# StuLiu/RegDA

Measured on AMD Instinct MI355X. Metric: src+tgt 512x512 image-pairs/sec (SSL step), higher is better.
Workload: dtype bf16; 1 GPU; st.regda.2potsdam SSL step, resnet101 DeepLabV2(PPM), batch 8+8 512x512 per GPU, online EMA teacher; global_batch=8, parallelism=dp1

## Files before the change

regda_amd/csrc/conv_kernels.hip:

```cpp
#include <stdio.h>
#include <stdlib.h>
#include <string.h>

#include "common.h"
#include <type_traits>
#include <vector>

struct ConvArgs {
    const bf16_t* x;
    const bf16_t* w;
    bf16_t* y;
    const bf16_t* res;
    rgda_stat_t* stats;
    int ldx, ldy, ldres;
    int N, H, W, Cin, Ho, Wo, Cout, KH, KW, stride, pad, dil, mode;
    int M;
    int tiles_c, tiles_p;
    int rows_per_group;
    int howo_shift, wo_shift;
    unsigned long long* dbg;
    int tpw;
    int skip;
    const unsigned char* res_mask;
    const bf16_t* bn_y;
// ... 1509 lines not shown
    const int nj1 = (t + 256) / SWP, nx1 = (t + 256) % SWP;
    const bool second = t + 256 < 2 * SWP;
    float na0[3] = {0.f, 0.f, 0.f}, na1[3] = {0.f, 0.f, 0.f}, nb0[3] = {0.f, 0.f, 0.f}, nb1[3] = {0.f, 0.f, 0.f};
    if (1 < rpw) {
        load_px(7 + nj0, nx0, na0);
        if (second) load_px(7 + nj1, nx1, na1);
    }
    float s[8], q[8];
#pragma unroll
    for (int e = 0; e < 8; ++e) { s[e] = 0.f; q[e] = 0.f; }
    EpiParams P;
    epilogue_params<KIND>(a, ((n * Ho + ho0) * Wo + wo0), (t % (BC / 8)) * 8, true, P);
    for (int r = 0; r < rpw; ++r) {
        const int ho = ho0 + r;
        asm volatile("s_waitcnt lgkmcnt(0)" ::: "memory");
        __builtin_amdgcn_s_barrier();
        if (r + 2 < rpw) {
            load_px(2 * r + 9 + nj0, nx0, nb0);
            if (second) load_px(2 * r + 9 + nj1, nx1, nb1);
        }
        f32x16 acc[1][1], acc1;
#pragma unroll
        for (int e = 0; e < 16; ++e) { acc[0][0][e] = 0.f; acc1[e] = 0.f; }
        const int px = wp * 32 + lrow;
        const unsigned char* fbase = srow + px * 16 + lk * 16;
        const int s0 = (2 * r) % 7;
#pragma unroll
        for (int kh = 0; kh < 7; ++kh) {
            const int slot = (s0 + kh >= 7) ? s0 + kh - 7 : s0 + kh;
            const bf16x8 fb0 = *(const bf16x8*)(fbase + slot * SROW);
            const bf16x8 fb1 = *(const bf16x8*)(fbase + slot * SROW + 32);
            acc[0][0] = __builtin_amdgcn_mfma_f32_32x32x16_bf16(fa[kh][0], fb0, acc[0][0], 0, 0, 0);
            acc1 = __builtin_amdgcn_mfma_f32_32x32x16_bf16(fa[kh][1], fb1, acc1, 0, 0, 0);
        }
#pragma unroll
        for (int e = 0; e < 16; ++e) acc[0][0][e] += acc1[e];
        const int m0 = (n * Ho + ho) * Wo + wo0;
        conv_epilogue<BC, BP, WC, WP, true, KIND>(a, acc, se, m0, 0, s, q, r + 1 == rpw, blockIdx.x & (NREP - 1), &P);
        if (r + 1 < rpw) {
            store_px(2 * r + 7 + nj0, nx0, na0);
            if (second) store_px(2 * r + 7 + nj1, nx1, na1);
        }
#pragma unroll
        for (int c = 0; c < 3; ++c) { na0[c] = nb0[c]; na1[c] = nb1[c]; }
    }
#endif
}

static int stem_conv_launch(const float* img, const void* wgt, void* y, int ldy, rgda_stat_t* stats, int stat_groups,
                            const BnEvalFuse* bne, int N, int H, int W, int Ho, int Wo, rgda_stream_t stream) {
    if (!img || !wgt || !y || N <= 0 || H <= 0 || W <= 0 || (ldy & 7) || ldy < 64) return RGDA_ERR_ARG;
    if (Ho != (H + 6 - 7) / 2 + 1 || Wo != (W + 6 - 7) / 2 + 1) return RGDA_ERR_ARG;
    if (Wo % 64) return RGDA_ERR_UNSUPPORTED;
    if ((long long)3 * H * W >= (1ll << 28)) return RGDA_ERR_UNSUPPORTED;
    if (stat_groups < 1) stat_groups = 1;
    if ((N % stat_groups) || (bne && stats)) return RGDA_ERR_ARG;
    const long long M = (long long)N * Ho * Wo;
    if (M > 0x7fffffffLL) return RGDA_ERR_ARG;
    ConvArgs a;
    a.x = nullptr; a.w = (const bf16_t*)wgt; a.y = (bf16_t*)y; a.res = nullptr; a.stats = stats; a.res_mask = nullptr;
    a.ldx = 0; a.ldy = ldy; a.ldres = 0;
    a.N = N; a.H = H; a.W = W; a.Cin = 3; a.Ho = Ho; a.Wo = Wo; a.Cout = 64; a.KH = 7; a.KW = 7;
    a.stride = 2; a.pad = 3; a.dil = 1; a.mode = 0;
    a.M = (int)M; a.tiles_c = 1; a.tiles_p = 0;
    a.rows_per_group = (int)(M / stat_groups);
    a.howo_shift = a.wo_shift = -1; a.dbg = nullptr; a.tpw = 0; a.skip = 0;
    a.bn_y = a.bn_x = nullptr; a.bn_mask = nullptr; a.bn_mi = a.bn_nscale = nullptr; a.bn_ldy = a.bn_ldx = a.bn_rpi = a.bn_relu = 0;
    a.bn_gamma = a.bn_beta = nullptr; a.xf.stats = nullptr;
    a.ev_rm = a.ev_rv = a.ev_gamma = a.ev_beta = nullptr; a.ev_eps = 0.f; a.ev_relu = 0;
    if (bne) {
        if (!bne->rm || !bne->rv || !bne->gamma || !bne->beta) return RGDA_ERR_ARG;
        a.ev_rm = bne->rm; a.ev_rv = bne->rv; a.ev_gamma = bne->gamma; a.ev_beta = bne->beta; a.ev_eps = bne->eps; a.ev_relu = bne->relu;
    }
    int rpw = 8;
    if (const char* e = TUNE_ENV("RGDA_STEM_RPW")) rpw = atoi(e);
    else while (rpw < 64 && (long long)N * (Ho / (2 * rpw)) * (Wo / 64) >= 512 && !(Ho % (2 * rpw))) rpw *= 2;
    while (rpw > 1 && (Ho % rpw)) rpw >>= 1;
    const long long blocks = (long long)N * (Ho / rpw) * (Wo / 64);
    if (blocks > 0x7fffffffLL) return RGDA_ERR_ARG;
    if (bne) stem_conv_kernel<EPI_EV><<<(int)blocks, 256, 0, to_stream(stream)>>>(a, img, rpw);
    else if (stats) stem_conv_kernel<EPI_STATS><<<(int)blocks, 256, 0, to_stream(stream)>>>(a, img, rpw);
    else stem_conv_kernel<EPI_PLAIN><<<(int)blocks, 256, 0, to_stream(stream)>>>(a, img, rpw);
    RGDA_CHECK_LAUNCH();
    return RGDA_OK;
}

__global__ void __launch_bounds__(256) stem_wgrad_kernel(const float* __restrict__ img, const bf16_t* __restrict__ dy, int lddy,
                                                         float* __restrict__ part, int H, int W, int Ho, int Wo, int rpw) {
#if defined(__HIP_DEVICE_COMPILE__)
    constexpr int BP = 64, KP = 192;
    constexpr int SWP = 136, SROW = SWP * 8, NSLOT = 9;
    constexpr int DT = 64 * 128;
    __shared__ __attribute__((aligned(256))) unsigned char smem[2 * DT + NSLOT * SROW];
    unsigned char* const sd = smem;
    unsigned char* const srow = smem + 2 * DT;

    const int t = threadIdx.x, lane = t & 63;
    const int wave = __builtin_amdgcn_readfirstlane(t >> 6);
    const int wi = wave & 1, wj = wave >> 1;
    const int wtiles = Wo / BP, rblocks = Ho / rpw;
    const int wo0 = (blockIdx.x % wtiles) * BP;
    const int ho0 = ((blockIdx.x / wtiles) % rblocks) * rpw, n = blockIdx.x / (wtiles * rblocks);
    const int hbase = ho0 * 2 - 3;

    const size_t plane = (size_t)H * W;
    const float* const img_n = img + (size_t)n * 3 * plane;
    auto load_px = [&](int j, int x, float (&v)[3]) {
        const int hi = hbase + j, wcol = wo0 * 2 - 3 + x;
        const bool ok = (unsigned)hi < (unsigned)H && (unsigned)wcol < (unsigned)W && x < 134;
        const size_t o = (size_t)(ok ? hi : 0) * W + (ok ? wcol : 0);
#pragma unroll
        for (int c = 0; c < 3; ++c) v[c] = ok ? img_n[c * plane + o] : 0.f;
    };
    auto store_px = [&](int j, int x, const float (&v)[3]) {
        uint2 p;
        p.x = pack2bf(v[0], v[1]);
        p.y = pack2bf(v[2], 0.f);
        *(uint2*)(srow + (j % NSLOT) * SROW + x * 8) = p;
    };
    const int dpx = t >> 2, dq = t & 3;
    auto load_dy = [&](int ho, uint4& v0, uint4& v1) {
        const bf16_t* dp = dy + ((size_t)(n * Ho + ho) * Wo + wo0 + dpx) * lddy + dq * 16;
        v0 = *(const uint4*)dp;
        v1 = *(const uint4*)(dp + 8);
    };
    auto store_dy = [&](int buf, const uint4& v0, const uint4& v1) {
        const int f = (dpx >> 1) & 1, s0 = dq * 2, s1 = dq * 2 + 1;
        unsigned char* b = sd + buf * DT + dpx * 128;
        *(uint4*)(b + ((((s0 >> 2) ^ f) << 6) | ((s0 & 3) << 4))) = v0;
        *(uint4*)(b + ((((s1 >> 2) ^ f) << 6) | ((s1 & 3) << 4))) = v1;
    };
#pragma unroll
    for (int i = 0; i < 4; ++i) {
        const int idx = t + 256 * i;
        if (idx < 7 * SWP) {
            float v[3];
            load_px(idx / SWP, idx % SWP, v);
            store_px(idx / SWP, idx % SWP, v);
        }
    }
    {
        uint4 v0, v1;
        load_dy(ho0, v0, v1);
        store_dy(0, v0, v1);
    }
    const int nj0 = t / SWP, nx0 = t % SWP;
    const int nj1 = (t + 256) / SWP, nx1 = (t + 256) % SWP;
    const bool second = t + 256 < 2 * SWP;
    float na0[3] = {0.f, 0.f, 0.f}, na1[3] = {0.f, 0.f, 0.f}, nb0[3] = {0.f, 0.f, 0.f}, nb1[3] = {0.f, 0.f, 0.f};
    if (1 < rpw) {
        load_px(7 + nj0, nx0, na0);
        if (second) load_px(7 + nj1, nx1, na1);
    }
    const int g = lane >> 4, la = lane & 15;
    const int krow = (g >> 1) * 8 + (la >> 2);
    const int kcol2 = ((g & 1) * 16 + (la & 3) * 4) * 2;
    auto pack_tr = [](s16x4 lo, s16x4 hi) {
        u16x8 v8 = {(bf16_t)lo[0], (bf16_t)lo[1], (bf16_t)lo[2], (bf16_t)lo[3],
                    (bf16_t)hi[0], (bf16_t)hi[1], (bf16_t)hi[2], (bf16_t)hi[3]};
        return __builtin_bit_cast(bf16x8, v8);
    };
    auto tr_dy = [&](const unsigned char* base, int byte, int r0) {
        const int r1 = r0 + 4;
        const unsigned char* p0 = base + r0 * 128 + ((((byte >> 6) ^ ((r0 >> 1) & 1)) << 6) | (byte & 63));
        const unsigned char* p1 = base + r1 * 128 + ((((byte >> 6) ^ ((r1 >> 1) & 1)) << 6) | (byte & 63));
        return pack_tr(__builtin_amdgcn_ds_read_tr16_b64_v4i16((s16x4 __attribute__((address_space(3)))*)(p0)),
                       __builtin_amdgcn_ds_read_tr16_b64_v4i16((s16x4 __attribute__((address_space(3)))*)(p1)));
    };
    auto tr_img = [&](const unsigned char* rowbase, int r0) {
        const unsigned char* p0 = rowbase + r0 * 16 + kcol2;
        return pack_tr(__builtin_amdgcn_ds_read_tr16_b64_v4i16((s16x4 __attribute__((address_space(3)))*)(p0)),
                       __builtin_amdgcn_ds_read_tr16_b64_v4i16((s16x4 __attribute__((address_space(3)))*)(p0 + 64)));
    };
    f32x16 acc[4];
#pragma unroll
    for (int j = 0; j < 4; ++j)
#pragma unroll
        for (int e = 0; e < 16; ++e) acc[j][e] = 0.f;
    const int kh0 = wj * 4, nkh = wj ? 3 : 4;

    for (int r = 0; r < rpw; ++r) {
        asm volatile("s_waitcnt lgkmcnt(0)" ::: "memory");
        __builtin_amdgcn_s_barrier();
        uint4 dv0 = uint4{0u, 0u, 0u, 0u}, dv1 = dv0;
        if (r + 1 < rpw) load_dy(ho0 + r + 1, dv0, dv1);
        if (r + 2 < rpw) {
            load_px(2 * r + 9 + nj0, nx0, nb0);
            if (second) load_px(2 * r + 9 + nj1, nx1, nb1);
        }
        const unsigned char* sdc = sd + (r & 1) * DT;
        const int s0 = (2 * r + kh0) % NSLOT;
#pragma unroll
        for (int kk = 0; kk < 4; ++kk) {
            const int r0 = kk * 16 + krow;
            const bf16x8 af = tr_dy(sdc, wi * 64 + kcol2, r0);
#pragma unroll
            for (int a = 0; a < 4; ++a) {
                if (a < nkh) {
                    const int slot = (s0 + a >= NSLOT) ? s0 + a - NSLOT : s0 + a;
                    const bf16x8 bf = tr_img(srow + slot * SROW, r0);
                    acc[a] = __builtin_amdgcn_mfma_f32_32x32x16_bf16(af, bf, acc[a], 0, 0, 0);
                }
            }
        }
        if (r + 1 < rpw) {
            store_dy((r + 1) & 1, dv0, dv1);
            store_px(2 * r + 7 + nj0, nx0, na0);
            if (second) store_px(2 * r + 7 + nj1, nx1, na1);
        }
#pragma unroll
        for (int c = 0; c < 3; ++c) { na0[c] = nb0[c]; na1[c] = nb1[c]; }
    }
    float* out = part + (size_t)blockIdx.x * 64 * KP;
    const int lrow = lane & 31, lk = lane >> 5;
    const int kw = lrow >> 2, c = lrow & 3;
    if (kw < 7 && c < 3) {
#pragma unroll
        for (int a = 0; a < 4; ++a)
            if (a < nkh) {
                const int k = ((kh0 + a) * 7 + kw) * 3 + c;
#pragma unroll
                for (int g4 = 0; g4 < 4; ++g4)
#pragma unroll
                    for (int e = 0; e < 4; ++e)
                        out[(wi * 32 + 8 * g4 + 4 * lk + e) * KP + k] = acc[a][4 * g4 + e];
            }
    }
#endif
}

__global__ void __launch_bounds__(256) stem_wgrad_reduce_kernel(const float* __restrict__ part, int nwg, float* __restrict__ dw) {
    __shared__ float red[8][32];
    const int o = blockIdx.x * 32 + (threadIdx.x & 31), sl = threadIdx.x >> 5;
    float a0 = 0.f, a1 = 0.f;
    if (o < 64 * 147) {
        const float* p = part + (size_t)(o / 147) * 192 + o % 147;
        int wg = sl;
        for (; wg + 8 < nwg; wg += 16) { a0 += p[(size_t)wg * 64 * 192]; a1 += p[(size_t)(wg + 8) * 64 * 192]; }
        if (wg < nwg) a0 += p[(size_t)wg * 64 * 192];
    }
    red[sl][threadIdx.x & 31] = a0 + a1;
    __syncthreads();
    if (threadIdx.x < 32 && o < 64 * 147) {
        float tot = 0.f;
#pragma unroll
        for (int i = 0; i < 8; ++i) tot += red[i][threadIdx.x];
        dw[o] += tot;
    }
}

static int stem_wgrad_rows(int N, int Ho, int Wo) {
    int rpw = 32;
    while (rpw > 1 && ((Ho % rpw) || (long long)N * (Ho / rpw) * (Wo / 64) < 512)) rpw >>= 1;
    return rpw;
}

extern "C" size_t rgda_stem_wgrad_workspace(int N, int H, int W) {
    if (N <= 0 || H <= 0 || W <= 0) return 0;
    const int Ho = (H + 6 - 7) / 2 + 1, Wo = (W + 6 - 7) / 2 + 1;
    if ((Wo % 64) || (long long)3 * H * W >= (1ll << 28)) return 0;
    return (size_t)N * (Ho / stem_wgrad_rows(N, Ho, Wo)) * (Wo / 64) * 64 * 192 * sizeof(float);
}

extern "C" int rgda_stem_wgrad(const float* img, const void* dy, int lddy, float* dw, void* ws, size_t ws_bytes, int N,
                               int H, int W, int Ho, int Wo, rgda_stream_t stream) {
    if (!img || !dy || !dw || !ws || N <= 0 || H <= 0 || W <= 0 || (lddy & 7) || lddy < 64) return RGDA_ERR_ARG;
    if (Ho != (H + 6 - 7) / 2 + 1 || Wo != (W + 6 - 7) / 2 + 1) return RGDA_ERR_ARG;
    if (Wo % 64) return RGDA_ERR_UNSUPPORTED;
    if ((long long)3 * H * W >= (1ll << 28)) return RGDA_ERR_UNSUPPORTED;
    if (((uintptr_t)ws & 15) || ws_bytes < rgda_stem_wgrad_workspace(N, H, W)) return RGDA_ERR_WORKSPACE;
    const int rpw = stem_wgrad_rows(N, Ho, Wo);
    const long long blocks = (long long)N * (Ho / rpw) * (Wo / 64);
    if (blocks > 0x7fffffffLL || (long long)N * Ho * Wo > 0x7fffffffLL) return RGDA_ERR_ARG;
    hipStream_t st = to_stream(stream);
    stem_wgrad_kernel<<<(int)blocks, 256, 0, st>>>(img, (const bf16_t*)dy, lddy, (float*)ws, H, W, Ho, Wo, rpw);
    RGDA_CHECK_LAUNCH();
    stem_wgrad_reduce_kernel<<<cdiv(64 * 147, 32), 256, 0, st>>>((const float*)ws, (int)blocks, dw);
    RGDA_CHECK_LAUNCH();
    return RGDA_OK;
}

extern "C" int rgda_stem_conv(const float* img, const void* wgt, void* y, int ldy, rgda_stat_t* stats, int stat_groups,
                              int N, int H, int W, int Ho, int Wo, rgda_stream_t stream) {
    return stem_conv_launch(img, wgt, y, ldy, stats, stat_groups, nullptr, N, H, W, Ho, Wo, stream);
}

extern "C" int rgda_stem_conv_bneval(const float* img, const void* wgt, void* y, int ldy, const float* running_mean,
                                     const float* running_var, const float* gamma, const float* beta, float eps, int relu,
                                     int N, int H, int W, int Ho, int Wo, rgda_stream_t stream) {
    BnEvalFuse e = {running_mean, running_var, gamma, beta, eps, relu};
    return stem_conv_launch(img, wgt, y, ldy, nullptr, 1, &e, N, H, W, Ho, Wo, stream);
}

struct WgradArgs {
    const bf16_t* x;
    const bf16_t* dy;
    float* dw;
    int ldx, lddy;
    int N, H, W, Cin, Ho, Wo, Cout, KH, KW, stride, pad, dil;
    int M;
    int tiles_co, tiles_ci, splits, kt_per_split;
    int howo_shift, wo_shift;
    int tap_fused;
    int lddw;
    int co_shift, co_nsub;
    float* ws_part;
    int* ws_cnt;
    unsigned long long* dbg;
};

typedef __attribute__((ext_vector_type(4))) unsigned u32x4;
#define RGDA_AUX_SC1 16
#define RGDA_SPLIT_GROUP 8
static inline __host__ __device__ int split_groups(int splits) { return splits > 2 * RGDA_SPLIT_GROUP ? (splits + RGDA_SPLIT_GROUP - 1) / RGDA_SPLIT_GROUP : 1; }
static inline __host__ __device__ int split_slots(int splits) { const int g = split_groups(splits); return splits + (g > 1 ? g : 0); }

template <int NACC, int NT>
static __device__ __forceinline__ bool split_k_combine(const WgradArgs& a, int tile, int split, f32x16 (&acc)[NACC],
                                                       unsigned char* smem) {
#if defined(__HIP_DEVICE_COMPILE__)
    const int t = threadIdx.x;
    constexpr int SLICE_B = NACC * 16 * NT * 4;
    const int S = a.splits, NG = split_groups(S), slots = split_slots(S);
    const __amdgpu_buffer_rsrc_t rs = __builtin_amdgcn_make_buffer_rsrc(
        (void*)(a.ws_part + (size_t)tile * slots * (SLICE_B / 4)), 0, slots * SLICE_B, 0x00020000);
    int* cnt = a.ws_cnt + tile * (NG + 1);
    int* flag = (int*)smem;
    auto publish = [&](int slot, int* counter) {
#pragma unroll
        for (int q = 0; q < NACC; ++q)
#pragma unroll
            for (int g = 0; g < 4; ++g) {
                const u32x4 v = {__float_as_uint(acc[q][4 * g]), __float_as_uint(acc[q][4 * g + 1]),
                                 __float_as_uint(acc[q][4 * g + 2]), __float_as_uint(acc[q][4 * g + 3])};
                __builtin_amdgcn_raw_buffer_store_b128(v, rs, ((q * 4 + g) * NT + t) * 16, slot * SLICE_B, RGDA_AUX_SC1);
            }
        asm volatile("s_waitcnt vmcnt(0)" ::: "memory");
        __syncthreads();
        if (t == 0) *flag = atomicAdd(counter, 1);
        __syncthreads();
        const int before = *flag;
        __syncthreads();
        return before;
    };
    auto gather = [&](int first, int count) {
        constexpr int CH = (NACC <= 4) ? NACC : ((NACC % 3 == 0) ? 3 : 4);
        constexpr bool PAIR = NACC <= 4;
        static_assert(NACC % CH == 0, "accumulator count must divide into chunks");
#pragma unroll
        for (int q0 = 0; q0 < NACC; q0 += CH) {
#pragma unroll
            for (int q = q0; q < q0 + CH; ++q)
#pragma unroll
                for (int r = 0; r < 16; ++r) acc[q][r] = 0.f;
            for (int sp = first; sp < first + count; sp += (PAIR ? 2 : 1)) {
                u32x4 v[CH * 4], w[PAIR ? CH * 4 : 1];
                const bool two = PAIR && sp + 1 < first + count;
#pragma unroll
                for (int i = 0; i < CH * 4; ++i)
                    v[i] = __builtin_amdgcn_raw_buffer_load_b128(rs, ((q0 * 4 + i) * NT + t) * 16, sp * SLICE_B, RGDA_AUX_SC1);
                if constexpr (PAIR) {
                    if (two) {
#pragma unroll
                        for (int i = 0; i < CH * 4; ++i)
                            w[i] = __builtin_amdgcn_raw_buffer_load_b128(rs, ((q0 * 4 + i) * NT + t) * 16, (sp + 1) * SLICE_B, RGDA_AUX_SC1);
                    }
                }
#pragma unroll
                for (int i = 0; i < CH * 4; ++i) {
                    const int q = q0 + i / 4, g = i % 4;
#pragma unroll
                    for (int e = 0; e < 4; ++e) acc[q][4 * g + e] += __uint_as_float(v[i][e]);
                }
                if constexpr (PAIR) {
                    if (two) {
#pragma unroll
                        for (int i = 0; i < CH * 4; ++i) {
                            const int q = q0 + i / 4, g = i % 4;
#pragma unroll
                            for (int e = 0; e < 4; ++e) acc[q][4 * g + e] += __uint_as_float(w[i][e]);
                        }
                    }
                }
            }
        }
    };
    const int G1 = (NG > 1) ? RGDA_SPLIT_GROUP : S;
    const int grp = split / G1, gfirst = grp * G1, gsize = min(G1, S - gfirst);
    if (publish(split, cnt + 1 + grp) != gsize - 1) return false;
    gather(gfirst, gsize);
    if (t == 0) cnt[1 + grp] = 0;
    if (NG == 1) return true;
    if (publish(S + grp, cnt) != NG - 1) return false;
    gather(S, NG);
    if (t == 0) cnt[0] = 0;
    return true;
#else
    return false;
#endif
}

#define RGDA_WGRAD_MAXG 16
struct WgradGroup {
    int n;
    int remap;
    int first[RGDA_WGRAD_MAXG + 1];
    WgradArgs a[RGDA_WGRAD_MAXG];
};

template <int LD>
static __device__ __forceinline__ void wait_tiles_in_flight(int tiles) {
    switch (tiles) {
        case 0: WAIT_VMCNT(0); break;
        case 1: WAIT_VMCNT(LD); break;
        case 2: WAIT_VMCNT(2 * LD); break;
        case 3: WAIT_VMCNT(3 * LD); break;
        default: WAIT_VMCNT(4 * LD); break;
    }
}

template <int BCO, int BCI, int WI = 2, int WJ = 2, int STAGES = 3>
__global__ void __launch_bounds__(64 * WI * WJ) conv_wgrad_kernel(WgradGroup g) {
#if defined(__HIP_DEVICE_COMPILE__)
    constexpr int NW = WI * WJ;
    constexpr int FI = BCO / (32 * WI), FJ = BCI / (32 * WJ);
    static_assert(FI >= 1 && FJ >= 1, "wave grid too fine for the tile");
    constexpr int RA = BCO * 2, RB = BCI * 2;
    constexpr int TA = 64 * RA, TB = 64 * RB, TILE = TA + TB;
    constexpr int LA = TA / (1024 * NW), LB = TB / (1024 * NW);
    static_assert(LA >= 1 && LB >= 1, "too many waves for the tile");
    constexpr int LD = LA + LB;
    static_assert(STAGES >= 3 && STAGES <= 6 && LD * (STAGES - 2) < 64, "vmcnt is 6 bits");
    __shared__ __attribute__((aligned(256))) unsigned char smem[STAGES * TILE];

    const int t = threadIdx.x, lane = t & 63;
    const int wave = __builtin_amdgcn_readfirstlane(t >> 6);
    const int wi = wave % WI, wj = wave / WI;
    int bid = g.remap ? xcd_remap(blockIdx.x, gridDim.x) : (int)blockIdx.x, layer = 0;
    while (layer + 1 < g.n && bid >= g.first[layer + 1]) ++layer;
    bid -= g.first[layer];
    const WgradArgs& a = g.a[layer];
    const int taps = a.KH * a.KW;
    const int split = bid % a.splits; bid /= a.splits;
    const int tco = bid % a.tiles_co; bid /= a.tiles_co;
    const int tci = bid % a.tiles_ci;
    const int tap = bid / a.tiles_ci;
    const int kh = tap / a.KW, kw = tap % a.KW;
    const int co0 = tco * BCO, ci0 = tci * BCI;
    const int kt_beg = split * a.kt_per_split;
    const int kt_end = min(kt_beg + a.kt_per_split, (a.M + 63) >> 6);
    const bool pointwise = (taps == 1 && a.stride == 1 && a.pad == 0);

    constexpr int RPA = 1024 / RA, RPB = 1024 / RB;
    const int ra = lane / (RA / 16), pa = lane % (RA / 16);
    const int rb = lane / (RB / 16), pb = lane % (RB / 16);
    constexpr int OOB = (int)0x80000000;
    const i32x4 rs_a = dma_rsrc(a.dy, (unsigned)((((size_t)a.M - 1) * a.lddy + a.Cout) * 2));
    const i32x4 rs_b = dma_rsrc(a.x, (unsigned)((((size_t)a.N * a.H * a.W - 1) * a.ldx + a.Cin) * 2));
    auto swz = [](int row, int slot, int rowbytes) {
        int f = (rowbytes >= 256) ? (row & 3) : ((row >> 1) & 1);
        return (((slot >> 2) ^ f) << 2) | (slot & 3);
    };
    int avo[LA], brow[LB], bcolb[LB], bvo[LB];
#pragma unroll
    for (int i = 0; i < LA; ++i) {
        int row = (i * NW + wave) * RPA + ra;
        int col = co0 + swz(row, pa, RA) * 8;
        avo[i] = (col < a.Cout) ? ((row * a.lddy + col) * 2) : OOB;
    }
#pragma unroll
    for (int i = 0; i < LB; ++i) {
        brow[i] = (i * NW + wave) * RPB + rb;
        int col = ci0 + swz(brow[i], pb, RB) * 8;
        bcolb[i] = (col < a.Cin) ? col * 2 : OOB;
        bvo[i] = (col < a.Cin) ? ((brow[i] * a.ldx + col) * 2) : OOB;
    }
    auto issue = [&](int kt, int stage) {
        const int mb = kt << 6;
        unsigned char* ab = smem + stage * TILE + wave * 1024;
        const int so_a = mb * a.lddy * 2;
#pragma unroll
        for (int i = 0; i < LA; ++i)
            dma16_to_lds(rs_a, ab + i * 1024 * NW, avo[i], so_a);
        unsigned char* bb = ab + TA;
        if (pointwise) {
            const int so_b = mb * a.ldx * 2;
#pragma unroll
            for (int i = 0; i < LB; ++i)
                dma16_to_lds(rs_b, bb + i * 1024 * NW, bvo[i], so_b);
        } else {
#pragma unroll
            for (int i = 0; i < LB; ++i) {
                int m = mb + brow[i];
                int n, rem, ho, wo;
                if (a.howo_shift >= 0) { n = m >> a.howo_shift; rem = m & ((1 << a.howo_shift) - 1); }
                else { n = m / (a.Ho * a.Wo); rem = m % (a.Ho * a.Wo); }
                if (a.wo_shift >= 0) { ho = rem >> a.wo_shift; wo = rem & ((1 << a.wo_shift) - 1); }
                else { ho = rem / a.Wo; wo = rem % a.Wo; }
                int hi = ho * a.stride - a.pad + kh * a.dil, wi2 = wo * a.stride - a.pad + kw * a.dil;
                bool ok = (m < a.M) && (bcolb[i] != OOB) && hi >= 0 && hi < a.H && wi2 >= 0 && wi2 < a.W;
                int vo = ok ? (((n * a.H + hi) * a.W + wi2) * a.ldx * 2 + bcolb[i]) : OOB;
                dma16_to_lds(rs_b, bb + i * 1024 * NW, vo, 0);
            }
        }
    };

    f32x16 acc[FI][FJ];
#pragma unroll
    for (int i = 0; i < FI; ++i)
#pragma unroll
        for (int j = 0; j < FJ; ++j)
#pragma unroll
            for (int r = 0; r < 16; ++r) acc[i][j][r] = 0.f;

    unsigned long long tq0 = 0, tq1 = 0, tq2 = 0;
    if (TDBG(a)) tq0 = __builtin_readcyclecounter();
    if (kt_beg < kt_end) {
        const int g = lane >> 4, la = lane & 15;
        const int krow = (g >> 1) * 8 + (la >> 2);
        const int kcol2 = ((g & 1) * 16 + (la & 3) * 4) * 2;
        bf16x8 af[4][FI], bfr[4][FJ];
        auto tr_pair = [&](const unsigned char* base, int rowbytes, int byte, int r0) {
            const int r1 = r0 + 4;
            int f0 = (rowbytes >= 256) ? (r0 & 3) : ((r0 >> 1) & 1), f1 = (rowbytes >= 256) ? (r1 & 3) : ((r1 >> 1) & 1);
            const unsigned char* p0 = base + r0 * rowbytes + ((((byte >> 6) ^ f0) << 6) | (byte & 63));
            const unsigned char* p1 = base + r1 * rowbytes + ((((byte >> 6) ^ f1) << 6) | (byte & 63));
            s16x4 lo = __builtin_amdgcn_ds_read_tr16_b64_v4i16((s16x4 __attribute__((address_space(3)))*)(p0));
            s16x4 hi = __builtin_amdgcn_ds_read_tr16_b64_v4i16((s16x4 __attribute__((address_space(3)))*)(p1));
            u16x8 v8 = {(bf16_t)lo[0], (bf16_t)lo[1], (bf16_t)lo[2], (bf16_t)lo[3],
                        (bf16_t)hi[0], (bf16_t)hi[1], (bf16_t)hi[2], (bf16_t)hi[3]};
            return __builtin_bit_cast(bf16x8, v8);
        };
        auto read_half = [&](int st, int h) {
            const unsigned char* ab = smem + st * TILE;
            const unsigned char* bb = ab + TA;
#pragma unroll
            for (int kk = 2 * h; kk < 2 * h + 2; ++kk) {
                const int r0 = kk * 16 + krow;
#pragma unroll
                for (int i = 0; i < FI; ++i) af[kk][i] = tr_pair(ab, RA, (wi * (BCO / WI) + i * 32) * 2 + kcol2, r0);
#pragma unroll
                for (int j = 0; j < FJ; ++j) bfr[kk][j] = tr_pair(bb, RB, (wj * (BCI / WJ) + j * 32) * 2 + kcol2, r0);
            }
        };
        auto mfma_half = [&](int h) {
#pragma unroll
            for (int kk = 2 * h; kk < 2 * h + 2; ++kk)
#pragma unroll
                for (int i = 0; i < FI; ++i)
#pragma unroll
                    for (int j = 0; j < FJ; ++j)
                        acc[i][j] = __builtin_amdgcn_mfma_f32_32x32x16_bf16(af[kk][i], bfr[kk][j], acc[i][j], 0, 0, 0);
        };
        int stage = 0;
        if constexpr (STAGES == 3) {
#pragma unroll
            for (int s0 = 0; s0 < 3; ++s0)
                if (kt_beg + s0 < kt_end) issue(kt_beg + s0, s0);
            wait_tiles_in_flight<LD>(min(2, kt_end - 1 - kt_beg));
            __builtin_amdgcn_s_barrier();
            if (TDBG(a)) tq1 = __builtin_readcyclecounter();
            read_half(0, 0);
            for (int kt = kt_beg; kt + 1 < kt_end; ++kt) {
                const int nxt = (stage == 2) ? 0 : stage + 1;
                read_half(stage, 1);
                mfma_half(0);
                asm volatile("s_waitcnt lgkmcnt(0)" ::: "memory");
                wait_tiles_in_flight<LD>(min(1, kt_end - 2 - kt));
                __builtin_amdgcn_s_barrier();
                if (kt + 3 < kt_end) issue(kt + 3, stage);
                read_half(nxt, 0);
                mfma_half(1);
                stage = nxt;
            }
            read_half(stage, 1);
            mfma_half(0);
            mfma_half(1);
        } else {
#pragma unroll
            for (int s0 = 0; s0 < STAGES - 1; ++s0)
                if (kt_beg + s0 < kt_end) issue(kt_beg + s0, s0);
            for (int kt = kt_beg; kt < kt_end; ++kt) {
                wait_tiles_in_flight<LD>(min(STAGES - 2, kt_end - 1 - kt));
                __builtin_amdgcn_s_barrier();
                if (TDBG(a) && kt == kt_beg) tq1 = __builtin_readcyclecounter();
                if (kt + STAGES - 1 < kt_end) issue(kt + STAGES - 1, stage >= 1 ? stage - 1 : STAGES - 1);
                read_half(stage, 0);
                read_half(stage, 1);
                mfma_half(0);
                mfma_half(1);
                stage = (stage == STAGES - 1) ? 0 : stage + 1;
            }
        }
    }
    if (TDBG(a)) tq2 = __builtin_readcyclecounter();
    if (a.splits > 1 && a.ws_part) {
        __syncthreads();
        f32x16 (&flat)[FI * FJ] = *reinterpret_cast<f32x16 (*)[FI * FJ]>(&acc[0][0]);
        if (!split_k_combine<FI * FJ, 64 * NW>(a, (tap * a.tiles_ci + tci) * a.tiles_co + tco, split, flat, smem)) return;
    }
    const int lcol = lane & 31, lk = lane >> 5;
    const unsigned rstep = a.co_shift >= 0 ? (unsigned)a.co_nsub : 1u;
    const unsigned rs = rstep * (unsigned)(taps * a.lddw);
    const bool full = (co0 + BCO <= a.Cout) && (ci0 + BCI <= a.Cin);
#pragma unroll
    for (int i = 0; i < FI; ++i)
#pragma unroll
        for (int j = 0; j < FJ; ++j) {
            const int cob = co0 + wi * (BCO / WI) + i * 32 + 4 * lk;
            const int ci = ci0 + wj * (BCI / WJ) + j * 32 + lcol;
            const unsigned rowb = a.co_shift >= 0 ? (unsigned)((cob & ((1 << a.co_shift) - 1)) * a.co_nsub + (cob >> a.co_shift))
                                                  : (unsigned)cob;
            unsigned o = rowb * (unsigned)(taps * a.lddw) + (unsigned)(tap * a.lddw + ci);
            if (full) {
#pragma unroll
                for (int g4 = 0; g4 < 4; ++g4) {
#pragma unroll
                    for (int q = 0; q < 4; ++q) atomicAdd(a.dw + (o + q * rs), acc[i][j][g4 * 4 + q]);
                    o += 8 * rs;
                }
            } else if (ci < a.Cin) {
#pragma unroll
                for (int r = 0; r < 16; ++r) {
                    int co = cob + (r & 3) + 8 * (r >> 2);
                    if (co < a.Cout) atomicAdd(a.dw + (o + (unsigned)((r & 3) + 8 * (r >> 2)) * rs), acc[i][j][r]);
                }
            }
        }
    if (TDBG(a) && t == 0) {
        TDBG(a)[blockIdx.x * 4 + 0] = tq0; TDBG(a)[blockIdx.x * 4 + 1] = tq1;
        TDBG(a)[blockIdx.x * 4 + 2] = tq2; TDBG(a)[blockIdx.x * 4 + 3] = __builtin_readcyclecounter();
    }
#endif
}

template <int WT, int D, int STAGES>
static __device__ __forceinline__ void conv_wgrad3x3_body(const WgradGroup& g) {
#if defined(__HIP_DEVICE_COMPILE__)
    constexpr int R = 64 / WT;
    constexpr int HR = R + 2 * D, HC = WT + 2 * D;
    constexpr int NH = HR * HC, NG = (NH + 7) / 8, NHP = NG * 8;
    constexpr int TA = 64 * 128, TB = (NHP * 128 + 1023) / 1024 * 1024, TILE = TA + TB;
    constexpr int LA = 2, LB = (NG + 3) / 4;
    constexpr int LD = LA + LB;
    static_assert(STAGES == 2 || STAGES == 3, "ring of 2 (two workgroups per CU) or 3 stages");
    __shared__ __attribute__((aligned(256))) unsigned char smem[STAGES * TILE];

    const int t = threadIdx.x, lane = t & 63;
    const int wave = __builtin_amdgcn_readfirstlane(t >> 6);
    const int wi = wave & 1, wj = wave >> 1;
    int bid = g.remap ? xcd_remap(blockIdx.x, gridDim.x) : (int)blockIdx.x, layer = 0;
    while (layer + 1 < g.n && bid >= g.first[layer + 1]) ++layer;
    bid -= g.first[layer];
    const WgradArgs& a = g.a[layer];
    const int split = bid % a.splits; bid /= a.splits;
    const int tco = bid % a.tiles_co;
    const int tci = bid / a.tiles_co;
    const int co0 = tco * 64, ci0 = tci * 64;
    const int tpr = a.W / WT, tpi = tpr * (a.H / R);
    const int KT = a.N * tpi;
    const int kt_beg = split * a.kt_per_split, kt_end = min(kt_beg + a.kt_per_split, KT);
    constexpr int OOB = (int)0x80000000;
    const i32x4 rs_a = dma_rsrc(a.dy, (unsigned)((((size_t)a.M - 1) * a.lddy + a.Cout) * 2));
    const i32x4 rs_b = dma_rsrc(a.x, (unsigned)((((size_t)a.N * a.H * a.W - 1) * a.ldx + a.Cin) * 2));

    const int lr = lane >> 3, ls = lane & 7;
    auto swz = [](int row, int slot) { return (((slot >> 2) ^ ((row >> 1) & 1)) << 2) | (slot & 3); };
    int avo[LA];
#pragma unroll
    for (int i = 0; i < LA; ++i) {
        int row = (i * 4 + wave) * 8 + lr;
        int col = co0 + swz(row, ls) * 8;
        avo[i] = (col < a.Cout) ? ((row * a.lddy + col) * 2) : OOB;
    }
    int bhr[LB], bhc[LB], bcol[LB];
#pragma unroll
    for (int i = 0; i < LB; ++i) {
        int h = min(i * 4 + wave, NG - 1) * 8 + lr;
        int col = ci0 + swz(h, ls) * 8;
        bool ok = (h < NH) && (col < a.Cin);
        bhr[i] = ok ? (h / HC - D) : -100000;
        bhc[i] = h % HC - D;
        bcol[i] = col * 2;
    }
    auto issue = [&](int kt, int stage) {
        const int n = kt / tpi, rem = kt % tpi;
        const int y0 = (rem / tpr) * R, x0 = (rem % tpr) * WT;
        unsigned char* ab = smem + stage * TILE + wave * 1024;
        const int so_a = ((n * a.H + y0) * a.W + x0) * a.lddy * 2;
#pragma unroll
        for (int i = 0; i < LA; ++i)
            dma16_to_lds(rs_a, ab + i * 4096, avo[i], so_a);
        unsigned char* bb = smem + stage * TILE + TA;
#pragma unroll
        for (int i = 0; i < LB; ++i) {
            int y = y0 + bhr[i], x = x0 + bhc[i];
            bool ok = (y >= 0) && (y < a.H) && (x >= 0) && (x < a.W);
            int vo = ok ? (((n * a.H + y) * a.W + x) * a.ldx * 2 + bcol[i]) : OOB;
            dma16_to_lds(rs_b, bb + min(i * 4 + wave, NG - 1) * 1024, vo, 0);
        }
    };

    f32x16 acc[9];
#pragma unroll
    for (int q = 0; q < 9; ++q)
#pragma unroll
        for (int r = 0; r < 16; ++r) acc[q][r] = 0.f;

    if (kt_beg < kt_end) {
        issue(kt_beg, 0);
        if (STAGES == 3 && kt_beg + 1 < kt_end) issue(kt_beg + 1, 1);
        const int g = lane >> 4, la = lane & 15;
        const int klane = (g >> 1) * 8 + (la >> 2);
        const int cbyte = ((g & 1) * 16 + (la & 3) * 4) * 2;
        const int abyte = wi * 64 + cbyte, bbyte = wj * 64 + cbyte;
        auto tr = [&](const unsigned char* base, int row, int byte) {
            const unsigned char* p = base + row * 128 + ((((byte >> 6) ^ ((row >> 1) & 1)) << 6) | (byte & 63));
            return __builtin_amdgcn_ds_read_tr16_b64_v4i16((s16x4 __attribute__((address_space(3)))*)(p));
        };
        auto pack = [](s16x4 lo, s16x4 hi) {
            u16x8 v8 = {(bf16_t)lo[0], (bf16_t)lo[1], (bf16_t)lo[2], (bf16_t)lo[3],
                        (bf16_t)hi[0], (bf16_t)hi[1], (bf16_t)hi[2], (bf16_t)hi[3]};
            return __builtin_bit_cast(bf16x8, v8);
        };
        int stage = 0;
        for (int kt = kt_beg; kt < kt_end; ++kt) {
            if (STAGES == 3 && kt + 1 < kt_end) WAIT_VMCNT(LD); else WAIT_VMCNT(0);
            __builtin_amdgcn_s_barrier();
            if (kt + STAGES - 1 < kt_end) issue(kt + STAGES - 1, stage >= 1 ? stage - 1 : STAGES - 1);
            const unsigned char* ab = smem + stage * TILE;
            const unsigned char* bb = ab + TA;
#pragma unroll
            for (int kk = 0; kk < 4; ++kk) {
                constexpr int dummy = 0; (void)dummy;
                const int r_kk = (kk * 16) / WT, c_kk = (kk * 16) % WT;
                const int k0 = kk * 16 + klane;
                bf16x8 af = pack(tr(ab, k0, abyte), tr(ab, k0 + 4, abyte));
#pragma unroll
                for (int kh = 0; kh < 3; ++kh)
#pragma unroll
                    for (int kw = 0; kw < 3; ++kw) {
                        const int h0 = (r_kk + kh * D) * HC + c_kk + kw * D + klane;
                        bf16x8 bfr = pack(tr(bb, h0, bbyte), tr(bb, h0 + 4, bbyte));
                        acc[kh * 3 + kw] = __builtin_amdgcn_mfma_f32_32x32x16_bf16(af, bfr, acc[kh * 3 + kw], 0, 0, 0);
                    }
            }
            stage = (stage == STAGES - 1) ? 0 : stage + 1;
        }
    }
    if (a.splits > 1 && a.ws_part) {
        __syncthreads();
        if (!split_k_combine<9, 256>(a, tci * a.tiles_co + tco, split, acc, smem)) return;
    }
    const int lcol = lane & 31, lk = lane >> 5;
    const int ci = ci0 + wj * 32 + lcol;
    if (ci < a.Cin) {
#pragma unroll
        for (int q = 0; q < 9; ++q)
#pragma unroll
            for (int r = 0; r < 16; ++r) {
                int co = co0 + wi * 32 + (r & 3) + 8 * (r >> 2) + 4 * lk;
                if (co < a.Cout) atomicAdd(a.dw + ((size_t)co * 9 + q) * a.lddw + ci, acc[q][r]);
            }
    }
#endif
}
template <int WT, int D, int STAGES = 3>
__global__ void __launch_bounds__(256) __attribute__((amdgpu_waves_per_eu(2, 2))) conv_wgrad3x3_kernel(WgradGroup g) {
    conv_wgrad3x3_body<WT, D, STAGES>(g);
}
template <int WT, int D, int STAGES = 3>
__global__ void __launch_bounds__(256) conv_wgrad3x3_wide_kernel(WgradGroup g) {
    conv_wgrad3x3_body<WT, D, STAGES>(g);
}

#define WGRAD_ROUTES                                                                           \
    WGRAD(WK_G128_128, 512, 128 * 128, 512, 0, conv_wgrad_kernel, 128, 128, 2, 4, 3)           \
    WGRAD(WK_G128_64, 512, 128 * 64, 512, 1, conv_wgrad_kernel, 128, 64, 4, 2, 3)              \
    WGRAD(WK_G64_128, 512, 64 * 128, 512, 1, conv_wgrad_kernel, 64, 128, 2, 4, 3)              \
    WGRAD(WK_G64_64, 256, 64 * 64, 512, 1, conv_wgrad_kernel, 64, 64, 2, 2, 3)                 \
    WGRAD(WK_G256_128, 512, 256 * 128, 256, 0, conv_wgrad_kernel, 256, 128, 4, 2, 3)           \
    WGRAD(WK_F64_1, 256, 9 * 64 * 64, 256, 1, conv_wgrad3x3_wide_kernel, 64, 1, 3)             \
    WGRAD(WK_F64_2, 256, 9 * 64 * 64, 256, 1, conv_wgrad3x3_wide_kernel, 64, 2, 3)             \
    WGRAD(WK_F32_1, 256, 9 * 64 * 64, 512, 1, conv_wgrad3x3_kernel, 32, 1, 2)                  \
    WGRAD(WK_F32_2, 256, 9 * 64 * 64, 256, 1, conv_wgrad3x3_wide_kernel, 32, 2, 3)             \
    WGRAD(WK_F16_1, 256, 9 * 64 * 64, 512, 1, conv_wgrad3x3_kernel, 16, 1, 3)                  \
    WGRAD(WK_F16_2, 256, 9 * 64 * 64, 512, 1, conv_wgrad3x3_kernel, 16, 2, 2)
#define WGRAD(ID, BLOCK, SLICE, CAPACITY, REMAP, KERNEL, ...) ID,
enum { WGRAD_ROUTES WK_COUNT };
#undef WGRAD
#define WGRAD(ID, BLOCK, SLICE, CAPACITY, REMAP, KERNEL, ...) {#KERNEL "<" #__VA_ARGS__ ">", SLICE, CAPACITY, REMAP},
static const struct { const char* name; size_t slice_floats; int capacity, remap; } WGRAD_KINDS[WK_COUNT] = {WGRAD_ROUTES};
#undef WGRAD

#ifndef RGDA_TAPFUSED_MIN_TILES
#define RGDA_TAPFUSED_MIN_TILES 1
#endif
static int wgrad_prepare(const rgda_wgrad_desc& d, WgradArgs& a) {
    if (!d.x || !d.dy || !d.dw) return RGDA_ERR_ARG;
    if (d.N <= 0 || d.H <= 0 || d.W <= 0 || d.Ho <= 0 || d.Wo <= 0 || d.Cin <= 0 || d.Cout <= 0 || d.kh <= 0 || d.kw <= 0 ||
        d.stride <= 0 || d.dil <= 0 || d.pad < 0)
        return RGDA_ERR_ARG;
    if ((d.Cin & 7) || (d.Cout & 7) || (d.ldx & 7) || (d.lddy & 7) || d.ldx < d.Cin || d.lddy < d.Cout) return RGDA_ERR_ARG;
    a.x = (const bf16_t*)d.x; a.dy = (const bf16_t*)d.dy; a.dw = d.dw; a.ldx = d.ldx; a.lddy = d.lddy;
    a.N = d.N; a.H = d.H; a.W = d.W; a.Cin = d.Cin; a.Ho = d.Ho; a.Wo = d.Wo; a.Cout = d.Cout; a.KH = d.kh; a.KW = d.kw;
    a.stride = d.stride; a.pad = d.pad; a.dil = d.dil;
    a.lddw = d.lddw ? d.lddw : d.Cin;
    a.co_shift = -1; a.co_nsub = 1;
    if (a.lddw < d.Cin) return RGDA_ERR_ARG;
    if (d.co_split) {
        const int sh = ilog2_exact(d.co_split);
        if (sh < 5 || (d.Cout % d.co_split) || d.kh != 1 || d.kw != 1) return RGDA_ERR_ARG;
        a.co_shift = sh; a.co_nsub = d.Cout / d.co_split;
    }
    if ((long long)d.Cout * d.kh * d.kw * a.lddw > 0xffffffffLL) return RGDA_ERR_ARG;
    long long M = (long long)d.N * d.Ho * d.Wo;
    if (M > 0x7fffffffLL - 64) return RGDA_ERR_ARG;
    a.M = (int)M;
    a.howo_shift = ilog2_exact(d.Ho * d.Wo);
    a.wo_shift = ilog2_exact(d.Wo);
    a.dbg = nullptr;
    if (const char* e = TUNE_ENV("RGDA_CONV_DBG")) a.dbg = (unsigned long long*)strtoull(e, nullptr, 0);
    a.splits = 1; a.kt_per_split = 0; a.ws_part = nullptr; a.ws_cnt = nullptr;
    a.tap_fused = 0;
    if (d.kh == 3 && d.kw == 3 && d.stride == 1 && d.pad == d.dil && d.Ho == d.H && d.Wo == d.W &&
        cdiv(d.Cout, 64) * cdiv(d.Cin, 64) >= RGDA_TAPFUSED_MIN_TILES && !TUNE_ENV("RGDA_WGRAD_GENERIC")) {
        int wt = (d.W >= 64) ? 64 : d.W;
        if ((wt == 64 || wt == 32 || wt == 16) && (d.W % wt) == 0 && (d.H % (64 / wt)) == 0 && (d.dil == 1 || d.dil == 2)) {
            a.tap_fused = 1;
            a.tiles_co = cdiv(d.Cout, 64);
            a.tiles_ci = cdiv(d.Cin, 64);
            if (d.dil == 2) return wt == 64 ? WK_F64_2 : wt == 32 ? WK_F32_2 : WK_F16_2;
            return wt == 64 ? WK_F64_1 : wt == 32 ? WK_F32_1 : WK_F16_1;
        }
    }
    int bco = (d.Cout <= 64) ? 64 : 128, bci = (d.Cin <= 64) ? 64 : 128;
    const int big = tune_int("RGDA_WGRAD_BIG", 1);
    if (big && bci == 128 && d.Cout >= 256 && (d.Cout % 256) == 0) bco = 256;
    a.tiles_co = cdiv(d.Cout, bco);
    a.tiles_ci = cdiv(d.Cin, bci);
    if (bco == 256) return WK_G256_128;
    return (bco == 128) ? (bci == 128 ? WK_G128_128 : WK_G128_64) : (bci == 128 ? WK_G64_128 : WK_G64_64);
}

static inline int wgrad_tiles(const WgradArgs& a) {
    return a.tiles_co * a.tiles_ci * (a.tap_fused ? 1 : a.KH * a.KW);
}
static inline int wgrad_ktiles(const WgradArgs& a) {
    if (!a.tap_fused) return cdiv(a.M, 64);
    int wt = (a.W >= 64) ? 64 : a.W;
    return a.N * (a.H / (64 / wt)) * (a.W / wt);
}

#define RGDA_WGRAD_WS_COUNTERS (64 * 1024)

static size_t wgrad_plan_splits(int kind, WgradGroup& g, bool have_ws) {
    const int capacity = WGRAD_KINDS[kind].capacity;
    const int minkt = tune_int("RGDA_WGRAD_MINKT", 16), rule = tune_int("RGDA_WGRAD_RULE", 1);
    int best = 1;
    if (have_ws && rule == 0) {
        int total = 0;
        for (int l = 0; l < g.n; ++l) total += wgrad_tiles(g.a[l]);
        best = cdiv(capacity, total);
    } else if (have_ws) {
        long long best_cost = -1;
        for (int S = 1; S <= 512; S += (S < 16 ? 1 : 8)) {
            long long wgs = 0, steps = 0;
            for (int l = 0; l < g.n; ++l) {
                const int KT = wgrad_ktiles(g.a[l]);
                int sl = S;
                if (sl > KT / minkt) sl = KT / minkt;
                if (sl < 1) sl = 1;
                const int per = cdiv(KT, sl);
                wgs += (long long)wgrad_tiles(g.a[l]) * cdiv(KT, per);
                if (per > steps) steps = per;
            }
            const int walk = split_groups(S) > 1 ? RGDA_SPLIT_GROUP + split_groups(S) + 8 : S;
            const long long cost = (long long)cdiv(wgs, capacity) * (steps + (S > 1 ? 8 + 2 * walk : 0));
            if (best_cost < 0 || cost < best_cost) { best_cost = cost; best = S; }
        }
    }
    best = tune_int("RGDA_WGRAD_SPLITS", best);
    size_t floats = 0;
    int items = 0, tiles_before = 0;
    for (int l = 0; l < g.n; ++l) {
        WgradArgs& a = g.a[l];
        const int KT = wgrad_ktiles(a);
        int splits = best;
        if (splits > KT / minkt) splits = KT / minkt;
        if (splits < 1) splits = 1;
        a.kt_per_split = cdiv(KT, splits);
        a.splits = cdiv(KT, a.kt_per_split);
        g.first[l] = items;
        items += wgrad_tiles(a) * a.splits;
        a.ws_part = (float*)(uintptr_t)floats;
        a.ws_cnt = (int*)(uintptr_t)tiles_before;
        if (a.splits > 1) {
            floats += (size_t)wgrad_tiles(a) * split_slots(a.splits) * WGRAD_KINDS[kind].slice_floats;
            tiles_before += wgrad_tiles(a) * (split_groups(a.splits) + 1);
        }
    }
    for (int l = g.n; l <= RGDA_WGRAD_MAXG; ++l) g.first[l] = items;
    return floats * 4;
}

static int wgrad_launch(int kind, WgradGroup& g, void* ws, size_t ws_bytes, hipStream_t st) {
    const size_t need = wgrad_plan_splits(kind, g, ws != nullptr);
    int counters = 0;
    for (int l = 0; l < g.n; ++l)
        if (g.a[l].splits > 1) counters += wgrad_tiles(g.a[l]) * (split_groups(g.a[l].splits) + 1);
    if (need && (size_t)counters * 4 > RGDA_WGRAD_WS_COUNTERS) {
        wgrad_plan_splits(kind, g, false);
        return wgrad_launch(kind, g, nullptr, 0, st);
    }
    if (need && ws_bytes < RGDA_WGRAD_WS_COUNTERS + need) return RGDA_ERR_WORKSPACE;
    for (int l = 0; l < g.n; ++l) {
        WgradArgs& a = g.a[l];
        a.ws_part = (float*)((char*)ws + RGDA_WGRAD_WS_COUNTERS) + (size_t)(uintptr_t)a.ws_part;
        a.ws_cnt = (int*)ws + (size_t)(uintptr_t)a.ws_cnt;
        if (TUNE_ENV("RGDA_WGRAD_ATOMIC")) a.ws_part = nullptr;
    }
    const int items = g.first[RGDA_WGRAD_MAXG];
    g.remap = tune_int("RGDA_WGRAD_REMAP", WGRAD_KINDS[kind].remap);
    switch (kind) {
#define WGRAD(ID, BLOCK, SLICE, CAPACITY, REMAP, KERNEL, ...) case ID: KERNEL<__VA_ARGS__><<<items, BLOCK, 0, st>>>(g); break;
        WGRAD_ROUTES
#undef WGRAD
    }
    RGDA_CHECK_LAUNCH();
    return RGDA_OK;
}

template <typename F>
static int wgrad_for_each_launch(const rgda_wgrad_desc* descs, int n, F fn) {
    static thread_local WgradGroup groups[WK_COUNT];
    for (int k = 0; k < WK_COUNT; ++k) groups[k].n = 0;
    for (int i = 0; i < n; ++i) {
        WgradArgs a;
        int kind = wgrad_prepare(descs[i], a);
        if (kind < 0) return kind;
    }
    for (int i = 0; i < n; ++i) {
        WgradArgs a;
        int kind = wgrad_prepare(descs[i], a);
        WgradGroup& g = groups[kind];
        g.a[g.n++] = a;
        if (g.n == RGDA_WGRAD_MAXG) {
            int rc = fn(kind, g);
            if (rc != RGDA_OK) return rc;
            g.n = 0;
        }
    }
    for (int k = 0; k < WK_COUNT; ++k)
        if (groups[k].n) {
            int rc = fn(k, groups[k]);
            if (rc != RGDA_OK) return rc;
        }
    return RGDA_OK;
}

extern "C" const char* rgda_conv2d_wgrad_kernel(const rgda_wgrad_desc* d) {
    if (!d) return nullptr;
    WgradArgs a;
    const int kind = wgrad_prepare(*d, a);
    return (kind >= 0 && kind < WK_COUNT) ? WGRAD_KINDS[kind].name : nullptr;
}

extern "C" size_t rgda_conv2d_wgrad_workspace(const rgda_wgrad_desc* descs, int n) {
    if (n <= 0 || !descs) return RGDA_WGRAD_WS_COUNTERS;
    size_t most = 0;
    wgrad_for_each_launch(descs, n, [&](int kind, WgradGroup& g) {
        const size_t b = wgrad_plan_splits(kind, g, true);
        if (b > most) most = b;
        return (int)RGDA_OK;
    });
    return RGDA_WGRAD_WS_COUNTERS + most;
}

extern "C" int rgda_conv2d_wgrad_grouped(const rgda_wgrad_desc* descs, int n, void* ws, size_t ws_bytes, rgda_stream_t stream) {
    if (n < 0 || (n > 0 && !descs)) return RGDA_ERR_ARG;
    if (ws && (ws_bytes < RGDA_WGRAD_WS_COUNTERS || ((uintptr_t)ws & 15))) return RGDA_ERR_WORKSPACE;
    hipStream_t st = to_stream(stream);
    const int rc = wgrad_for_each_launch(descs, n, [&](int kind, WgradGroup& g) { return wgrad_launch(kind, g, ws, ws_bytes, st); });
    if (rc != RGDA_OK && ws) (void)hipMemsetAsync(ws, 0, RGDA_WGRAD_WS_COUNTERS, st);
    return rc;
}

extern "C" int rgda_conv2d_wgrad(const void* x, int ldx, const void* dy, int lddy, float* dw, int N, int H, int W,
                                 int Cin, int Ho, int Wo, int Cout, int kh, int kw, int stride, int pad, int dil,
                                 void* ws, size_t ws_bytes, rgda_stream_t stream) {
    const rgda_wgrad_desc d = {x, dy, dw, ldx, lddy, N, H, W, Cin, Ho, Wo, Cout, kh, kw, stride, pad, dil, 0, 0};
    return rgda_conv2d_wgrad_grouped(&d, 1, ws, ws_bytes, stream);
}
```

Before: 439.1 pairs/s.

## Split tap-fused 3x3 wgrad into per-kernel-row tiles for wide variants

For the 64-wide (dil 1 and 2) and 32-wide dil-2 tap-fused 3x3 weight-gradient kernels, each workgroup now computes a single kernel row (3 taps) instead of all 9, with the kernel row index taken from the block id. This triples the number of output tiles, cuts accumulator registers from 9 to 3 tiles and shrinks the input halo in LDS, aiming for better occupancy and more parallelism. In exchange, the dy tile is loaded three times across workgroups, and the split-k capacity and workspace slice sizes are adjusted to match.

```diff
diff --git a/regda_amd/csrc/conv_kernels.hip b/regda_amd/csrc/conv_kernels.hip
--- a/regda_amd/csrc/conv_kernels.hip
+++ b/regda_amd/csrc/conv_kernels.hip
@@ -1835,6 +1835,7 @@
     int tiles_co, tiles_ci, splits, kt_per_split;
     int howo_shift, wo_shift;
     int tap_fused;
+    int tap_tiles;
     int lddw;
     int co_shift, co_nsub;
     float* ws_part;
@@ -2167,11 +2168,21 @@
 #endif
 }
 
+#ifndef RGDA_WGRAD_ROWTILE
+#define RGDA_WGRAD_ROWTILE 3
+#endif
+static constexpr __host__ __device__ int wgrad3x3_tap_rows(int wt, int d) {
+    return ((wt == 64 && d == 1 && (RGDA_WGRAD_ROWTILE & 1)) || (wt == 64 && d == 2 && (RGDA_WGRAD_ROWTILE & 2)) ||
+            (wt == 32 && d == 2 && (RGDA_WGRAD_ROWTILE & 4))) ? 1 : 3;
+}
+
 template <int WT, int D, int STAGES>
 static __device__ __forceinline__ void conv_wgrad3x3_body(const WgradGroup& g) {
 #if defined(__HIP_DEVICE_COMPILE__)
     constexpr int R = 64 / WT;
-    constexpr int HR = R + 2 * D, HC = WT + 2 * D;
+    constexpr int TR = wgrad3x3_tap_rows(WT, D);
+    constexpr int NACC = 3 * TR;
+    constexpr int HR = R + (TR - 1) * D, HC = WT + 2 * D;
     constexpr int NH = HR * HC, NG = (NH + 7) / 8, NHP = NG * 8;
     constexpr int TA = 64 * 128, TB = (NHP * 128 + 1023) / 1024 * 1024, TILE = TA + TB;
     constexpr int LA = 2, LB = (NG + 3) / 4;
@@ -2186,6 +2197,8 @@
     while (layer + 1 < g.n && bid >= g.first[layer + 1]) ++layer;
     bid -= g.first[layer];
     const WgradArgs& a = g.a[layer];
+    int kh0 = 0;
+    if constexpr (TR == 1) { kh0 = bid % 3; bid /= 3; }
     const int split = bid % a.splits; bid /= a.splits;
     const int tco = bid % a.tiles_co;
     const int tci = bid / a.tiles_co;
@@ -2212,7 +2225,7 @@
         int h = min(i * 4 + wave, NG - 1) * 8 + lr;
         int col = ci0 + swz(h, ls) * 8;
         bool ok = (h < NH) && (col < a.Cin);
-        bhr[i] = ok ? (h / HC - D) : -100000;
+        bhr[i] = ok ? (h / HC + (kh0 - 1) * D) : -100000;
         bhc[i] = h % HC - D;
         bcol[i] = col * 2;
     }
@@ -2234,9 +2247,9 @@
         }
     };
 
-    f32x16 acc[9];
-#pragma unroll
-    for (int q = 0; q < 9; ++q)
+    f32x16 acc[NACC];
+#pragma unroll
+    for (int q = 0; q < NACC; ++q)
 #pragma unroll
         for (int r = 0; r < 16; ++r) acc[q][r] = 0.f;
 
@@ -2270,7 +2283,7 @@
                 const int k0 = kk * 16 + klane;
                 bf16x8 af = pack(tr(ab, k0, abyte), tr(ab, k0 + 4, abyte));
 #pragma unroll
-                for (int kh = 0; kh < 3; ++kh)
+                for (int kh = 0; kh < TR; ++kh)
 #pragma unroll
                     for (int kw = 0; kw < 3; ++kw) {
                         const int h0 = (r_kk + kh * D) * HC + c_kk + kw * D + klane;
@@ -2283,17 +2296,17 @@
     }
     if (a.splits > 1 && a.ws_part) {
         __syncthreads();
-        if (!split_k_combine<9, 256>(a, tci * a.tiles_co + tco, split, acc, smem)) return;
+        if (!split_k_combine<NACC, 256>(a, (tci * a.tiles_co + tco) * (3 / TR) + kh0, split, acc, smem)) return;
     }
     const int lcol = lane & 31, lk = lane >> 5;
     const int ci = ci0 + wj * 32 + lcol;
     if (ci < a.Cin) {
 #pragma unroll
-        for (int q = 0; q < 9; ++q)
+        for (int q = 0; q < NACC; ++q)
 #pragma unroll
             for (int r = 0; r < 16; ++r) {
                 int co = co0 + wi * 32 + (r & 3) + 8 * (r >> 2) + 4 * lk;
-                if (co < a.Cout) atomicAdd(a.dw + ((size_t)co * 9 + q) * a.lddw + ci, acc[q][r]);
+                if (co < a.Cout) atomicAdd(a.dw + ((size_t)co * 9 + kh0 * 3 + q) * a.lddw + ci, acc[q][r]);
             }
     }
 #endif
@@ -2307,16 +2320,18 @@
     conv_wgrad3x3_body<WT, D, STAGES>(g);
 }
 
+#define F3X3_SLICE(WT, D) (3 * wgrad3x3_tap_rows(WT, D) * 64 * 64)
+#define F3X3_CAPACITY(WT, D) (wgrad3x3_tap_rows(WT, D) == 1 ? 512 : 256)
 #define WGRAD_ROUTES                                                                           \
     WGRAD(WK_G128_128, 512, 128 * 128, 512, 0, conv_wgrad_kernel, 128, 128, 2, 4, 3)           \
     WGRAD(WK_G128_64, 512, 128 * 64, 512, 1, conv_wgrad_kernel, 128, 64, 4, 2, 3)              \
     WGRAD(WK_G64_128, 512, 64 * 128, 512, 1, conv_wgrad_kernel, 64, 128, 2, 4, 3)              \
     WGRAD(WK_G64_64, 256, 64 * 64, 512, 1, conv_wgrad_kernel, 64, 64, 2, 2, 3)                 \
     WGRAD(WK_G256_128, 512, 256 * 128, 256, 0, conv_wgrad_kernel, 256, 128, 4, 2, 3)           \
-    WGRAD(WK_F64_1, 256, 9 * 64 * 64, 256, 1, conv_wgrad3x3_wide_kernel, 64, 1, 3)             \
-    WGRAD(WK_F64_2, 256, 9 * 64 * 64, 256, 1, conv_wgrad3x3_wide_kernel, 64, 2, 3)             \
+    WGRAD(WK_F64_1, 256, F3X3_SLICE(64, 1), F3X3_CAPACITY(64, 1), 1, conv_wgrad3x3_wide_kernel, 64, 1, 3) \
+    WGRAD(WK_F64_2, 256, F3X3_SLICE(64, 2), F3X3_CAPACITY(64, 2), 1, conv_wgrad3x3_wide_kernel, 64, 2, 3) \
     WGRAD(WK_F32_1, 256, 9 * 64 * 64, 512, 1, conv_wgrad3x3_kernel, 32, 1, 2)                  \
-    WGRAD(WK_F32_2, 256, 9 * 64 * 64, 256, 1, conv_wgrad3x3_wide_kernel, 32, 2, 3)             \
+    WGRAD(WK_F32_2, 256, F3X3_SLICE(32, 2), F3X3_CAPACITY(32, 2), 1, conv_wgrad3x3_wide_kernel, 32, 2, 3) \
     WGRAD(WK_F16_1, 256, 9 * 64 * 64, 512, 1, conv_wgrad3x3_kernel, 16, 1, 3)                  \
     WGRAD(WK_F16_2, 256, 9 * 64 * 64, 512, 1, conv_wgrad3x3_kernel, 16, 2, 2)
 #define WGRAD(ID, BLOCK, SLICE, CAPACITY, REMAP, KERNEL, ...) ID,
@@ -2355,12 +2370,13 @@
     a.dbg = nullptr;
     if (const char* e = TUNE_ENV("RGDA_CONV_DBG")) a.dbg = (unsigned long long*)strtoull(e, nullptr, 0);
     a.splits = 1; a.kt_per_split = 0; a.ws_part = nullptr; a.ws_cnt = nullptr;
-    a.tap_fused = 0;
+    a.tap_fused = 0; a.tap_tiles = 1;
     if (d.kh == 3 && d.kw == 3 && d.stride == 1 && d.pad == d.dil && d.Ho == d.H && d.Wo == d.W &&
         cdiv(d.Cout, 64) * cdiv(d.Cin, 64) >= RGDA_TAPFUSED_MIN_TILES && !TUNE_ENV("RGDA_WGRAD_GENERIC")) {
         int wt = (d.W >= 64) ? 64 : d.W;
         if ((wt == 64 || wt == 32 || wt == 16) && (d.W % wt) == 0 && (d.H % (64 / wt)) == 0 && (d.dil == 1 || d.dil == 2)) {
             a.tap_fused = 1;
+            a.tap_tiles = 3 / wgrad3x3_tap_rows(wt, d.dil);
             a.tiles_co = cdiv(d.Cout, 64);
             a.tiles_ci = cdiv(d.Cin, 64);
             if (d.dil == 2) return wt == 64 ? WK_F64_2 : wt == 32 ? WK_F32_2 : WK_F16_2;
@@ -2377,7 +2393,7 @@
 }
 
 static inline int wgrad_tiles(const WgradArgs& a) {
-    return a.tiles_co * a.tiles_ci * (a.tap_fused ? 1 : a.KH * a.KW);
+    return a.tiles_co * a.tiles_ci * (a.tap_fused ? a.tap_tiles : a.KH * a.KW);
 }
 static inline int wgrad_ktiles(const WgradArgs& a) {
     if (!a.tap_fused) return cdiv(a.M, 64);
```

Measured after the change: 440.5 pairs/s (median of 6 runs). No clear change (+0.3%).
